# adalca/neurite

Measured on AMD Instinct MI355X. Metric: Mvoxels/sec interpn+Dice on 160^3 x 32-label, higher is better.
Workload: dtype f32

## Files before the change

### neurite_amd/csrc/fused.hip

```cpp

#include <stdio.h>
#include <stdlib.h>

#include <type_traits>

#include "dice_reduce.h"
#include "interpn_core.h"
#include "wc.h"
#include "fused_wc.h"

namespace {

typedef unsigned nrt_u2 __attribute__((ext_vector_type(2)));
template <typename ST> struct RowT;
template <> struct RowT<float> {
    typedef nrt_f4 T;
    static constexpr unsigned BYTES = 16;
    static __device__ __forceinline__ nrt_f4 widen(const nrt_f4 &t) { return t; }
};
template <> struct RowT<unsigned short> {
    typedef nrt_u2 T;
    static constexpr unsigned BYTES = 8;
    static __device__ __forceinline__ nrt_f4 widen(const nrt_u2 &t) {
        return (nrt_f4){__uint_as_float(t[0] << 16), __uint_as_float(t[0] & 0xffff0000u), __uint_as_float(t[1] << 16),
                        __uint_as_float(t[1] & 0xffff0000u)};
    }
};


constexpr int FUSED_SYNC = 8;
constexpr int FUSED_MINW = 3;

template <bool BY_VALUE, typename T> using BodyArg = std::conditional_t<BY_VALUE, const T, const T &>;
template <int G, int MODE, bool STORE, typename ST, bool PAD>
__device__ __forceinline__ void warp_dice_tile_body(BodyArg<PAD && MODE == NRT_LOC_LINSPACE && STORE, InterpArgs> a,
                                                    BodyArg<PAD && !std::is_same<ST, float>::value, TileGeom> tg,
                                                    const void *__restrict__ fixed,
                                                    float *__restrict__ fpart, float *__restrict__ mpart, int Gr_arg) {
    typedef typename RowT<ST>::T Row;
    constexpr unsigned RB = RowT<ST>::BYTES;
    constexpr int NG = 256 / G;
    constexpr int LP = 4 * G;
    const int Gr = PAD ? Gr_arg : G;
    const int L = 4 * Gr;
    const unsigned k = blockIdx.x % NRT_NXCD, jb = blockIdx.x / NRT_NXCD;
    unsigned per = tg.per2 * tg.nTz;
    unsigned nb = gridDim.x / NRT_NXCD;
    int b = blockIdx.y;
    unsigned ucol = 0, prow = blockIdx.x;
    XmWork xw = {};
// ... 237 lines not shown
    if (t == 0 && G == 8 && xmarch_applies(out_shape, batch)) {
        t = xmarch_default_tune();
        tile_geometry(out_shape, G, t, t, tg, nblocks);
    }
    if (((t >> 14) & 1) && !tg.plane_major) {
        int lty = tg.lty;
        while ((1 << (lty + tg.ltz)) < 256 / G) ++lty;
        if (lty != tg.lty) {
            t = (t & ~((15 << 4) | (15 << 8))) | (lty << 4) | (tg.ltz << 8);
            tile_geometry(out_shape, G, t, t, tg, nblocks);
        }
    }
    if (nblocks > (unsigned)DICE_MAX_BLOCKS) nblocks = DICE_MAX_BLOCKS;
    if (((t >> 14) & 1) && !tg.plane_major && out_shape[0] > 0) {
        unsigned grid;
        if (((t >> 16) & 0xff) == 0) nblocks = xmarch_setup_mixed(out_shape, batch, t, tg, grid);
        else nblocks = xmarch_setup(out_shape, batch, t, tg);
    }
}

constexpr int FUSED_TUNE_WC = 1 << 29, FUSED_TUNE_NO_WC = 1 << 30;

struct FusedChoice { bool wc, persist; };
inline FusedChoice fused_choose(const InterpArgs &a, const TileGeom &tg, int G, bool f32_storage, bool allow_wc) {
    FusedChoice c = {false, false};
    if (G == 8 && f32_storage && allow_wc && wc_applies(tg, G, a)) {
        c.wc = true;
        c.persist = wc_persistent(tg);
    }
    return c;
}

template <typename... P, typename... A>
int launch_kernel(void (*kern)(P...), dim3 grid, unsigned dyn, hipStream_t st, A... args) {
    if (dyn && hipFuncSetAttribute((const void *)kern, hipFuncAttributeMaxDynamicSharedMemorySize, (int)dyn) != hipSuccess)
        return NRT_ERR_LAUNCH;
    hipLaunchKernelGGL(kern, grid, dim3(256), dyn, st, args...);
    return NRT_OK;
}

template <int G, int MODE, bool STORE, int MINW, typename ST, bool PAD>
int launch_tile(dim3 grid, unsigned dyn, hipStream_t st, const InterpArgs &a, const TileGeom &tg, const void *fixed, float *fpart,
                float *mpart, int Gr) {
    if constexpr (PAD) return launch_kernel(warp_dice_tile_pad<G, MODE, STORE, MINW, ST>, grid, dyn, st, a, tg, fixed, fpart, mpart, Gr);
    else return launch_kernel(warp_dice_tile<G, MODE, STORE, MINW, ST>, grid, dyn, st, a, tg, fixed, fpart, mpart);
}

template <int G, typename ST, bool PAD>
int launch_fused(const InterpArgs &a, const TileGeom &tg, unsigned nblocks, int batch, int mode, bool store, int Gr,
                 const void *fixed, float *fpart, float *mpart, hipStream_t st, bool allow_wc, bool want_minmax) {
    if constexpr (G == 8 && std::is_same<ST, float>::value && !PAD) {
        if (fused_choose(a, tg, G, true, allow_wc).wc)
            return launch_wc(a, tg, nblocks, batch, mode, store, want_minmax, (const float *)fixed, fpart, mpart, st);
    }
    const dim3 grid = tg.x_march ? dim3(fused_xmarch_grid(tg, nblocks, batch), 1) : dim3(nblocks, batch);
    const unsigned dyn = tg.x_march && !store ? 75u * 1024u : 0u;
#define NRT_FUSED(MODE)                                                                                                          \
    return tg.x_march ? (store ? launch_tile<G, MODE, true, FUSED_MINW, ST, PAD>(grid, dyn, st, a, tg, fixed, fpart, mpart, Gr)  \
                               : launch_tile<G, MODE, false, FUSED_MINW, ST, PAD>(grid, dyn, st, a, tg, fixed, fpart, mpart, Gr)) \
                      : (store ? launch_tile<G, MODE, true, 1, ST, PAD>(grid, dyn, st, a, tg, fixed, fpart, mpart, Gr)           \
                               : launch_tile<G, MODE, false, 1, ST, PAD>(grid, dyn, st, a, tg, fixed, fpart, mpart, Gr))
    switch (mode) {
        case NRT_LOC_ABSOLUTE: NRT_FUSED(NRT_LOC_ABSOLUTE);
        case NRT_LOC_SHIFT: NRT_FUSED(NRT_LOC_SHIFT);
        default: NRT_FUSED(NRT_LOC_LINSPACE);
    }
#undef NRT_FUSED
}

template <int G, typename ST, typename... A>
int launch_fused_any(int Gr, const A &...args) {
    if constexpr (G > 1) {
        if (Gr != G) return launch_fused<G, ST, true>(args...);
    }
    return launch_fused<G, ST, false>(args...);
}
// ... 125 lines not shown
```

### neurite_amd/csrc/fused_wc.h

```cpp

#pragma once

#include <type_traits>

#include "dice_reduce.h"
#include "interpn_core.h"

namespace {

#ifndef WC_NST_WARP
#define WC_NST_WARP 3
#endif
#ifndef WC_NST_FUSED
#define WC_NST_FUSED 2
#endif
#ifndef WC_NST_BWD
#define WC_NST_BWD 3
#endif
#ifndef WC_FIXED_GROUPS
#define WC_FIXED_GROUPS 4
#endif
constexpr int WC_SLOTS = 128;
constexpr int WC_OVF = 16;
constexpr int WC_TRASH_ROW = WC_SLOTS + WC_OVF;
constexpr int WC_ROWS = WC_TRASH_ROW + 1;
constexpr unsigned WC_NOROW = 0x01ffffffu;
constexpr unsigned WC_TAGS_OFF = WC_ROWS * 128;
constexpr unsigned WC_LIST_OFF = WC_TAGS_OFF + 528;
constexpr unsigned WC_BC_OFF = WC_LIST_OFF + 512;
constexpr unsigned WC_WAVE_BYTES = WC_BC_OFF + 128;
constexpr unsigned WC_BLOCK_BYTES = 4 * WC_WAVE_BYTES;
static_assert(WC_LIST_OFF % 16 == 0 && WC_BC_OFF % 16 == 0 && WC_WAVE_BYTES % 16 == 0, "LDS layout");
static_assert((WC_SLOTS + 1) * 4 <= 528 && WC_ROWS <= 256, "LDS layout");
static_assert(2 * WC_BLOCK_BYTES <= 160 * 1024, "two blocks per CU");

typedef __attribute__((address_space(3))) char wc_lds_char;
typedef __attribute__((address_space(3))) nrt_f4 wc_lds_f4;
typedef __attribute__((address_space(3))) volatile nrt_i4 wc_lds_vi4;
typedef __attribute__((address_space(3))) volatile unsigned wc_lds_vu32;
typedef unsigned wc_u3 __attribute__((ext_vector_type(3)));
typedef unsigned wc_u4 __attribute__((ext_vector_type(4)));
typedef float wc_f3 __attribute__((ext_vector_type(3)));

__device__ __forceinline__ void wc_corner(float pv, float mx, int &i0, int &i1, float &w0) {
    const float cl = fminf(fmaxf(pv, 0.0f), mx);
    const float l0 = floorf(cl);
    const float l1 = fminf(nrt_add(l0, 1.0f), mx);
    i0 = (int)l0; i1 = (int)l1;
    w0 = nrt_sub(l1, cl);
}

__device__ __forceinline__ __amdgpu_buffer_rsrc_t wc_rsrc(const void *base, unsigned bytes) {
    const unsigned long long v = (unsigned long long)base;
    const void *u = (const void *)(((unsigned long long)(unsigned)__builtin_amdgcn_readfirstlane((unsigned)(v >> 32)) << 32) |
                                   (unsigned long long)(unsigned)__builtin_amdgcn_readfirstlane((unsigned)v));
    return __builtin_amdgcn_make_buffer_rsrc((void *)u, 0, __builtin_amdgcn_readfirstlane((int)bytes), 0x00020000);
}

struct WcBwd {
    const float *sums, *gdice;
    float eps;
    float *gloc;
};

template <int MODE, bool STORE, bool MM, bool FILL, bool DICE, int BWD = 0>
__device__ __forceinline__ void wc_item(const InterpArgs &a, const TileGeom &tg, const float *__restrict__ fixed, float *__restrict__ fpart,
                                        float *__restrict__ mpart, const XmWork &xw, char *wc_smem, const WcBwd &bw = WcBwd{nullptr, nullptr, 0.0f, nullptr}) {
    constexpr int G = 8, L = 32;
    static_assert(BWD == 0 || (DICE && !STORE && !MM), "the backward form reads a second row per voxel and stores the location gradient only");
    const int b = __builtin_amdgcn_readfirstlane(xw.b);
    const unsigned prow = (unsigned)__builtin_amdgcn_readfirstlane((int)xw.prow), ucol = (unsigned)__builtin_amdgcn_readfirstlane((int)xw.ucol);
    const unsigned RY = 1u << tg.lry, RZ = 1u << tg.lrz;
    const unsigned nRz = (tg.nTz + RZ - 1) / RZ;
    const unsigned reg = ucol / (RY * RZ), wr = ucol % (RY * RZ);
    const unsigned cy = (reg / nRz) * RY + wr / RZ, cz = (reg % nRz) * RZ + wr % RZ;
    const int x0 = __builtin_amdgcn_readfirstlane(xw.x0), y0 = (int)cy << 2, z0 = (int)cz << 3;
    int npass = __builtin_amdgcn_readfirstlane(xw.xlen);
    if (cy >= tg.nTy || cz >= tg.nTz || npass < 0) npass = 0;

    const int lane = threadIdx.x & 63, wave = threadIdx.x >> 6;
    const int g = lane >> 3, p = lane & 7;
    const int dzt = (0x1320 >> ((g & 3) * 4)) & 15;
    const int yy = y0 + 2 * (wave >> 1) + (g >> 2), zz = z0 + 4 * (wave & 1) + dzt;
    const bool yzvalid = (yy < a.O[1]) && (zz < a.O[2]);
    const int yc = min(yy, a.O[1] - 1), zc = min(zz, a.O[2] - 1);
    const unsigned qyz = (unsigned)yc * (unsigned)a.O[2] + (unsigned)zc, qstep = (unsigned)a.O[1] * (unsigned)a.O[2];
    const unsigned SY = (unsigned)a.S[1], SZ = (unsigned)a.S[2];
    const float mxx = (float)(a.S[0] - 1), mxy = (float)(a.S[1] - 1), mxz = (float)(a.S[2] - 1);
    const float fyc = (float)yc, fzc = (float)zc;
    const float ly = (yc == 0) ? 0.0f : ((yc == a.O[1] - 1) ? mxy : nrt_mul(a.delta[1], fyc));
    const float lz = (zc == 0) ? 0.0f : ((zc == a.O[2] - 1) ? mxz : nrt_mul(a.delta[2], fzc));

    const char *volb = (const char *)a.vol + (long long)b * a.vol_bs * 4ll;
    const unsigned long long volbytes = (unsigned long long)a.S[0] * SY * SZ * 128ull;
    const unsigned outbytes = a.nout * 128u;
    const __amdgpu_buffer_rsrc_t vres = wc_rsrc(volb, (unsigned)volbytes);
    const __amdgpu_buffer_rsrc_t lres = wc_rsrc(MODE != NRT_LOC_LINSPACE ? (const char *)(a.loc + (long long)b * a.loc_bs) : volb, a.nout * 12u);
    const __amdgpu_buffer_rsrc_t fres = wc_rsrc(DICE ? (const char *)fixed + (long long)b * a.out_bs * 4ll : volb, outbytes);
    const __amdgpu_buffer_rsrc_t ores = wc_rsrc(STORE ? (const char *)a.out + (long long)b * a.out_bs * 4ll : volb, outbytes);
    const __amdgpu_buffer_rsrc_t gres = wc_rsrc(BWD ? (const char *)(bw.gloc + (long long)b * a.nout * 3) : volb, a.nout * 12u);
    const unsigned gl_lane = (p == 0 && yzvalid) ? qyz * 12u : 0xffffffffu;
    float ca[4] = {0.0f, 0.0f, 0.0f, 0.0f}, cb[4] = {0.0f, 0.0f, 0.0f, 0.0f};
    if (BWD == 1) {
        const float *sm = bw.sums + (long long)b * 3 * L;
#pragma unroll
        for (int k = 0; k < 4; ++k) {
            const int l = p * 4 + k;
            const float num = 2.0f * sm[l] + bw.eps, den = sm[L + l] + sm[2 * L + l] + bw.eps;
            const float gd = bw.gdice[(long long)b * L + l];
            if (den != 0.0f) { ca[k] = 2.0f * gd / den; cb[k] = -2.0f * gd * num / (den * den); }
        }
    }
    const unsigned loc_lane = qyz * 12u, row_lane = (qyz * 8u + (unsigned)p) * 16u;
    const unsigned out_lane = yzvalid ? row_lane : 0xffffffffu;
    const unsigned loc_step = qstep * 12u, row_step = qstep * 128u;
    const unsigned p16 = (unsigned)p * 16u;

    wc_lds_char *wl = (wc_lds_char *)wc_smem + wave * WC_WAVE_BYTES;
    wc_lds_vu32 *tags = (wc_lds_vu32 *)(wl + WC_TAGS_OFF);
    wc_lds_char *lrow = wl + p * 16;
    tags[lane] = ~0u;
    tags[lane + 64] = ~0u;
    const bool cx1 = (p & 4) != 0, cy1 = (p & 2) != 0, cz1 = (p & 1) != 0;

    nrt_f2 stp_l = {0, 0}, stp_h = {0, 0}, stt_l = {0, 0}, stt_h = {0, 0}, spp_l = {0, 0}, spp_h = {0, 0};
    float mnt = INFINITY, mxt = -INFINITY, mnp = INFINITY, mxp = -INFINITY;

    constexpr int FG = WC_FIXED_GROUPS, NX = 8 - FG;
    static_assert(FG == 3 || FG == 4, "WC_FIXED_GROUPS");
    struct Pass {
        float w0x, w0y, w0z;
        unsigned sl[8];
        unsigned lr[FG], ld[FG];
        unsigned xr[NX], xd[NX];
        int n;
        int xq;
        float mk[3];
        bool oob;
        nrt_f4 T;
        nrt_f4 F[FG], Fx[NX];
        float pn[3];
    };
    struct Mg { float w0x, w0y, w0z; bool oob, miss; unsigned rid, slot, t1, t2, mytag; float mk[3]; };
    constexpr int NST = ((BWD ? WC_NST_BWD : (DICE ? WC_NST_FUSED : WC_NST_WARP)) > 2) ? 3 : 2;
    constexpr bool XSH = NST == 3 && DICE;
    Pass A, B, C;
    nrt_f4 FxS[NX];
#pragma unroll
    for (int i = 0; i < NX; ++i) FxS[i] = (nrt_f4){0.f, 0.f, 0.f, 0.f};
    auto reset = [&](Pass &s) {
        s.w0x = s.w0y = s.w0z = 0.f; s.n = 0; s.xq = x0; s.oob = false; s.mk[0] = s.mk[1] = s.mk[2] = 0.f;
        s.T = (nrt_f4){0.f, 0.f, 0.f, 0.f};
#pragma unroll
        for (int i = 0; i < FG; ++i) { s.F[i] = (nrt_f4){0.f, 0.f, 0.f, 0.f}; s.lr[i] = WC_NOROW << 7; s.ld[i] = WC_TRASH_ROW * 128u; }
#pragma unroll
        for (int i = 0; i < NX; ++i) { s.Fx[i] = (nrt_f4){0.f, 0.f, 0.f, 0.f}; s.xr[i] = WC_NOROW << 7; s.xd[i] = WC_TRASH_ROW * 128u; }
#pragma unroll
        for (int i = 0; i < 8; ++i) s.sl[i] = 0;
        s.pn[0] = s.pn[1] = s.pn[2] = 0.f;
    };
    reset(A); reset(B);
    if (NST == 3) reset(C);

    auto fetch_loc = [&](int pass, Pass &s) {
        if (MODE != NRT_LOC_LINSPACE) {
            const wc_u3 v = __builtin_bit_cast(wc_u3, __builtin_amdgcn_raw_buffer_load_b96(lres, loc_lane, (unsigned)(x0 + pass) * loc_step, 0));
            s.pn[0] = __uint_as_float(v[0]); s.pn[1] = __uint_as_float(v[1]); s.pn[2] = __uint_as_float(v[2]);
        }
    };
    auto fetch_row = [&](unsigned rowoff) -> nrt_f4 {
        return __builtin_bit_cast(nrt_f4, __builtin_amdgcn_raw_buffer_load_b128(vres, rowoff | p16, 0, 0));
    };

    auto m1a = [&](int pass, const Pass &s, Mg &m) {
        const int xq = x0 + pass;
        float px, py, pz;
        if (MODE == NRT_LOC_ABSOLUTE) { px = s.pn[0]; py = s.pn[1]; pz = s.pn[2]; }
        else if (MODE == NRT_LOC_SHIFT) { px = nrt_add((float)xq, s.pn[0]); py = nrt_add(fyc, s.pn[1]); pz = nrt_add(fzc, s.pn[2]); }
        else { px = (xq == 0) ? 0.0f : ((xq == a.O[0] - 1) ? mxx : nrt_mul(a.delta[0], (float)xq)); py = ly; pz = lz; }
        int i0x, i1x, i0y, i1y, i0z, i1z;
        wc_corner(px, mxx, i0x, i1x, m.w0x);
        wc_corner(py, mxy, i0y, i1y, m.w0y);
        wc_corner(pz, mxz, i0z, i1z, m.w0z);
        m.oob = FILL ? ((px < 0.0f) || (px > mxx) || (py < 0.0f) || (py > mxy) || (pz < 0.0f) || (pz > mxz)) : false;
        if (BWD) {
            m.mk[0] = (fminf(fmaxf(px, 0.0f), mxx) == px) ? 1.0f : 0.0f;
            m.mk[1] = (fminf(fmaxf(py, 0.0f), mxy) == py) ? 1.0f : 0.0f;
            m.mk[2] = (fminf(fmaxf(pz, 0.0f), mxz) == pz) ? 1.0f : 0.0f;
        }
        const unsigned ix = cx1 ? i1x : i0x, iy = cy1 ? i1y : i0y, iz = cz1 ? i1z : i0z;
        m.rid = nrt_mad24(nrt_mad24(ix, SY, iy), SZ, iz);
        m.slot = ((ix & 3u) << 5) | ((iy & 3u) << 3) | (iz & 7u);
        m.mytag = (m.rid << 6) | (unsigned)lane;
        m.t1 = tags[m.slot];
// ... 6 lines not shown
    auto m1c = [&](int pass, const Mg &m, Pass &s) {
        const unsigned x2 = m.t2 ^ m.mytag;
        const bool served = x2 < 64u;
        const bool loader = m.miss && x2 == 0u;
        const bool orphan = !served;
        const unsigned long long Ml = __builtin_amdgcn_ballot_w64(loader), Mo = __builtin_amdgcn_ballot_w64(orphan);
        const unsigned long long Mf = Ml | Mo;
        const int no = __builtin_popcountll(Mo);
        int n = __builtin_popcountll(Mf);
        const unsigned ro = __builtin_amdgcn_mbcnt_hi((unsigned)(Mo >> 32), __builtin_amdgcn_mbcnt_lo((unsigned)Mo, 0u));
        const unsigned rf = __builtin_amdgcn_mbcnt_hi((unsigned)(Mf >> 32), __builtin_amdgcn_mbcnt_lo((unsigned)Mf, 0u));
        bool fetcher = loader || orphan;
        unsigned src = orphan ? (unsigned)WC_SLOTS + ro : m.slot;
        unsigned e = fetcher ? rf : (unsigned)n + ((unsigned)lane - rf);
        if (__builtin_expect(no > WC_OVF, 0)) {
            tags[lane] = ~0u;
            tags[lane + 64] = ~0u;
            e = (unsigned)lane; fetcher = true; src = (unsigned)lane; n = 64;
        }
        const unsigned src128 = src * 128u;
        const unsigned tp = ((e & 7u) << 3) | (e >> 3);
        typedef unsigned wc_u2 __attribute__((ext_vector_type(2)));
        *(__attribute__((address_space(3))) volatile wc_u2 *)(wl + WC_LIST_OFF + tp * 8u) =
            (wc_u2){fetcher ? (m.rid << 7) : (WC_NOROW << 7), fetcher ? src128 : (unsigned)WC_TRASH_ROW * 128u};
        ((__attribute__((address_space(3))) volatile unsigned short *)(wl + WC_BC_OFF))[lane] = (unsigned short)src128;
        const nrt_i4 la = *(wc_lds_vi4 *)(wl + WC_LIST_OFF + g * 64), lb = *(wc_lds_vi4 *)(wl + WC_LIST_OFF + g * 64 + 16);
        const nrt_i4 sh = *(wc_lds_vi4 *)(wl + WC_BC_OFF + g * 16);
        s.lr[0] = (unsigned)la[0]; s.ld[0] = (unsigned)la[1]; s.lr[1] = (unsigned)la[2]; s.ld[1] = (unsigned)la[3];
        s.lr[2] = (unsigned)lb[0]; s.ld[2] = (unsigned)lb[1];
        if (FG == 4) { s.lr[FG - 1] = (unsigned)lb[2]; s.ld[FG - 1] = (unsigned)lb[3]; }
        else { s.xr[0] = (unsigned)lb[2]; s.xd[0] = (unsigned)lb[3]; }
        if (__builtin_expect(n > 32, 0)) {
            const nrt_i4 lc = *(wc_lds_vi4 *)(wl + WC_LIST_OFF + g * 64 + 32), le = *(wc_lds_vi4 *)(wl + WC_LIST_OFF + g * 64 + 48);
            s.xr[NX - 4] = (unsigned)lc[0]; s.xd[NX - 4] = (unsigned)lc[1]; s.xr[NX - 3] = (unsigned)lc[2]; s.xd[NX - 3] = (unsigned)lc[3];
            s.xr[NX - 2] = (unsigned)le[0]; s.xd[NX - 2] = (unsigned)le[1]; s.xr[NX - 1] = (unsigned)le[2]; s.xd[NX - 1] = (unsigned)le[3];
        }
#pragma unroll
        for (int c = 0; c < 4; ++c) { s.sl[2 * c] = (unsigned)sh[c] & 0xffffu; s.sl[2 * c + 1] = (unsigned)sh[c] >> 16; }
        s.w0x = m.w0x; s.w0y = m.w0y; s.w0z = m.w0z; s.oob = m.oob;
        s.n = __builtin_amdgcn_readfirstlane(n);
        if (BWD) { s.mk[0] = m.mk[0]; s.mk[1] = m.mk[1]; s.mk[2] = m.mk[2]; }
        s.xq = x0 + pass;
    };
    auto issue = [&](Pass &s) {
#pragma unroll
        for (int i = 0; i < FG; ++i) s.F[i] = fetch_row(s.lr[i]);
        if (!XSH && __builtin_expect(s.n > 8 * FG, 0)) {
#pragma unroll
            for (int i = 0; i < NX; ++i)
                if (i == 0 || s.n > 8 * (FG + i)) s.Fx[i] = fetch_row(s.xr[i]);
        }
        if (DICE) s.T = __builtin_bit_cast(nrt_f4, __builtin_amdgcn_raw_buffer_load_b128(fres, row_lane, (unsigned)s.xq * row_step, 2));
    };
    auto issue_x = [&](Pass &s) {
        if (XSH && __builtin_expect(s.n > 8 * FG, 0)) {
#pragma unroll
            for (int i = 0; i < NX; ++i)
                if (i == 0 || s.n > 8 * (FG + i)) FxS[i] = fetch_row(s.xr[i]);
        }
    };
    auto deliver = [&](Pass &s) {
        *(wc_lds_f4 *)(lrow + s.ld[0]) = s.F[0];
#pragma unroll
        for (int i = 1; i < FG; ++i)
            if (s.n > 8 * i) *(wc_lds_f4 *)(lrow + s.ld[i]) = s.F[i];
        if (__builtin_expect(s.n > 8 * FG, 0)) {
#pragma unroll
            for (int i = 0; i < NX; ++i)
                if (i == 0 || s.n > 8 * (FG + i)) *(wc_lds_f4 *)(lrow + s.xd[i]) = XSH ? FxS[i] : s.Fx[i];
        }
    };

    const int last = npass - 1;
    auto step = [&](int pass, Pass &s, Pass &o, Pass &nx, auto masked) {
        constexpr bool MASKED = decltype(masked)::value;
        issue(o);
        __builtin_amdgcn_sched_barrier(0);
        deliver(s);
        nrt_f4 R[8];
#pragma unroll
        for (int corner = 0; corner < 8; ++corner) R[corner] = *(const wc_lds_f4 *)(lrow + s.sl[corner]);
        __builtin_amdgcn_sched_barrier(0);
        Mg m;
        m1a(min(pass + NST, last), s, m);
        __builtin_amdgcn_sched_barrier(0);
        const float w1x = nrt_sub(1.0f, s.w0x), w1y = nrt_sub(1.0f, s.w0y), w1z = nrt_sub(1.0f, s.w0z);
        const nrt_f2 wy2 = {s.w0y, w1y}, wz2 = {s.w0z, w1z};
        const nrt_f2 wxy0 = (nrt_f2){s.w0x, s.w0x} * wy2, wxy1 = (nrt_f2){w1x, w1x} * wy2;
        nrt_f2 wt2[4];
        wt2[0] = (nrt_f2){wxy0[0], wxy0[0]} * wz2;
        wt2[1] = (nrt_f2){wxy0[1], wxy0[1]} * wz2;
        wt2[2] = (nrt_f2){wxy1[0], wxy1[0]} * wz2;
// ... 9 lines not shown
        }
        asm volatile("" : "+v"(al), "+v"(ah));
        __builtin_amdgcn_sched_barrier(0);
        m1b(m);
        __builtin_amdgcn_sched_barrier(0);
#pragma unroll
        for (int corner = 4; corner < (BLEND ? 8 : 4); ++corner) {
            const float wt = wt2[corner >> 1][corner & 1];
            const nrt_f2 w2 = {wt, wt};
            al = al + w2 * (nrt_f2){R[corner][0], R[corner][1]};
            ah = ah + w2 * (nrt_f2){R[corner][2], R[corner][3]};
        }
        nrt_f4 acc = {al[0], al[1], ah[0], ah[1]};
        const unsigned xqcur = (unsigned)s.xq;
        const float cw0x = s.w0x, cw0y = s.w0y, cw0z = s.w0z, cmx = s.mk[0], cmy = s.mk[1], cmz = s.mk[2];
        const bool coob = s.oob;
        if (!BWD) {
            if (FILL) {
#pragma unroll
                for (int c = 0; c < 4; ++c) acc[c] = apply_fill(acc[c], s.oob, a.fill_f);
            }
            if (STORE) __builtin_amdgcn_raw_buffer_store_b128(__builtin_bit_cast(wc_u4, acc), ores, out_lane, (unsigned)s.xq * row_step, 2);
        }
        const nrt_f4 Tcur = s.T;
        asm volatile("" : "+v"(acc));
        __builtin_amdgcn_sched_barrier(0);
        m1c(min(pass + NST, last), m, s);
        __builtin_amdgcn_sched_barrier(0);
        if (BWD) {
            nrt_f2 gl2 = {Tcur[0], Tcur[1]}, gh2 = {Tcur[2], Tcur[3]};
            if (BWD == 1) {
                gl2 = __builtin_elementwise_fma((nrt_f2){cb[0], cb[1]}, (nrt_f2){acc[0], acc[1]}, (nrt_f2){ca[0], ca[1]} * gl2);
                gh2 = __builtin_elementwise_fma((nrt_f2){cb[2], cb[3]}, (nrt_f2){acc[2], acc[3]}, (nrt_f2){ca[2], ca[3]} * gh2);
            }
            if (FILL && coob) { gl2 = (nrt_f2){0.0f, 0.0f}; gh2 = gl2; }
            float gacc[3];
            loc_grad_rows(R, gl2, gh2, cw0x, w1x, cw0y, w1y, cw0z, w1z, cmx, cmy, cmz, gacc);
#pragma unroll
            for (int d = 0; d < 3; ++d) {
                float r = gacc[d];
                r += __int_as_float(__builtin_amdgcn_update_dpp(0, __float_as_int(r), 0xB1, 0xF, 0xF, true));
                r += __int_as_float(__builtin_amdgcn_update_dpp(0, __float_as_int(r), 0x4E, 0xF, 0xF, true));
                r += __int_as_float(__builtin_amdgcn_update_dpp(0, __float_as_int(r), 0x141, 0xF, 0xF, true));
                gacc[d] = r;
            }
            __builtin_amdgcn_raw_buffer_store_b96(__builtin_bit_cast(wc_u3, (wc_f3){gacc[0], gacc[1], gacc[2]}), gres, gl_lane, xqcur * loc_step, 0);
        } else if (DICE) {
            nrt_f4 T = Tcur;
            if (MASKED) {
#pragma unroll
                for (int c = 0; c < 4; ++c) { T[c] = yzvalid ? T[c] : 0.0f; acc[c] = yzvalid ? acc[c] : 0.0f; }
// ... 57 lines not shown
        fetch_loc(min(2, last), A);
        m1a(min(1, last), B, m); m1b(m); m1c(min(1, last), m, B);
        fetch_loc(min(3, last), B);
        __builtin_amdgcn_sched_barrier(0);
        int pass = 0;
        if (npass >= 2) {
            step(0, A, B, B, masked);
            step(1, B, A, A, masked);
            for (pass = 2; pass + 1 < npass; pass += 2) {
                step(pass, A, B, B, masked);
                step(pass + 1, B, A, A, masked);
            }
        }
        if (pass < npass) step(pass, A, B, B, masked);
    };
    if (npass > 0) {
        if (DICE && !BWD && __builtin_amdgcn_ballot_w64(!yzvalid) != 0ull) march(std::true_type());
        else march(std::false_type());
    }

    if (!DICE || BWD) return;
    nrt_f4 stp = {stp_l[0], stp_l[1], stp_h[0], stp_h[1]}, stt = {stt_l[0], stt_l[1], stt_h[0], stt_h[1]},
           spp = {spp_l[0], spp_l[1], spp_h[0], spp_h[1]};
#pragma unroll
    for (int c = 0; c < 4; ++c) {
        stp[c] = wave_xor_add(stp[c], G);
        stt[c] = wave_xor_add(stt[c], G);
        spp[c] = wave_xor_add(spp[c], G);
    }
    for (int off = 1; off < NRT_WAVE; off <<= 1) {
        mnt = fminf(mnt, __shfl_xor(mnt, off, NRT_WAVE)); mxt = fmaxf(mxt, __shfl_xor(mxt, off, NRT_WAVE));
        mnp = fminf(mnp, __shfl_xor(mnp, off, NRT_WAVE)); mxp = fmaxf(mxp, __shfl_xor(mxp, off, NRT_WAVE));
    }
    __syncthreads();
    float (*red)[3 * L + 4] = (float (*)[3 * L + 4])wc_smem;
    if (lane < G) {
#pragma unroll
        for (int c = 0; c < 4; ++c) {
            red[wave][0 * L + 4 * lane + c] = stp[c];
            red[wave][1 * L + 4 * lane + c] = stt[c];
            red[wave][2 * L + 4 * lane + c] = spp[c];
        }
    }
    if (lane == 0) { red[wave][3 * L + 0] = mnt; red[wave][3 * L + 1] = mxt; red[wave][3 * L + 2] = mnp; red[wave][3 * L + 3] = mxp; }
    __syncthreads();
    const long long pbase = (long long)b * tg.prows + prow;
// ... 33 lines not shown
        if (jb == 0xffffffffu) break;
        XmWork xw;
        if (!xmarch_work_at(tg, O0, kk, jb, xw)) continue;
        item(xw);
    }
    if (threadIdx.x == 0 && atomicAdd(&queue[NRT_NXCD * 16u], 1u) == gridDim.x - 1) {
        for (unsigned q = 0; q <= NRT_NXCD; ++q) queue[q * 16u] = 0u;
    }
}

template <int MODE, bool STORE, bool MM, bool FILL, bool DICE = true, bool PERSIST = false>
__global__ __launch_bounds__(256, 2) void warp_dice_wc(InterpArgs a, TileGeom tg, const float *__restrict__ fixed,
                                                        float *__restrict__ fpart, float *__restrict__ mpart, unsigned *__restrict__ queue) {
    extern __shared__ __attribute__((aligned(16))) char wc_smem[];
    if (!PERSIST) {
        XmWork xw;
        if (!xmarch_work(tg, a.O[0], xw)) return;
        wc_item<MODE, STORE, MM, FILL, DICE>(a, tg, fixed, fpart, mpart, xw, wc_smem);
        return;
    }
    wc_persistent_loop(tg, a.O[0], queue, [&](const XmWork &xw) { wc_item<MODE, STORE, MM, FILL, DICE>(a, tg, fixed, fpart, mpart, xw, wc_smem); });
}

template <int MODE, bool FILL, int BWD, bool PERSIST>
__global__ __launch_bounds__(256, 2) void warp_dice_wc_bwd(InterpArgs a, TileGeom tg, const float *__restrict__ rows, WcBwd bw,
                                                            unsigned *__restrict__ queue) {
    extern __shared__ __attribute__((aligned(16))) char wc_smem[];
    if (!PERSIST) {
        XmWork xw;
        if (!xmarch_work(tg, a.O[0], xw)) return;
        wc_item<MODE, false, false, FILL, true, BWD>(a, tg, rows, nullptr, nullptr, xw, wc_smem, bw);
        return;
    }
    wc_persistent_loop(tg, a.O[0], queue, [&](const XmWork &xw) { wc_item<MODE, false, false, FILL, true, BWD>(a, tg, rows, nullptr, nullptr, xw, wc_smem, bw); });
}

inline bool wc_persistent(const TileGeom &tg) { return NRT_NXCD * tg.items_x > 2u * (unsigned)nrt_num_cus(); }
static_assert(NRT_RING_GATHER_OFF == 0 && (NRT_NXCD + 1) * 16 <= NRT_RING_CCE_OFF, "the work counters of a launch stay in the gather's words of a slot");

template <int MODE, bool STORE, bool MM, bool FILL>
int launch_wc_inst(const InterpArgs &a, const TileGeom &tg, unsigned nblocks, int batch, const float *fixed, float *fpart, float *mpart,
                   hipStream_t st) {
    const unsigned items = NRT_NXCD * tg.items_x, slots = 2u * (unsigned)nrt_num_cus();
    unsigned *queue = wc_persistent(tg) ? nrt_ring_slot(st) : nullptr;
    if (queue) {
        if (hipFuncSetAttribute((const void *)warp_dice_wc<MODE, STORE, MM, FILL, true, true>, hipFuncAttributeMaxDynamicSharedMemorySize,
                                (int)WC_BLOCK_BYTES) != hipSuccess)
            return NRT_ERR_LAUNCH;
        hipLaunchKernelGGL((warp_dice_wc<MODE, STORE, MM, FILL, true, true>), dim3(nrt_xcd_grid(slots)), dim3(256), WC_BLOCK_BYTES, st, a, tg, fixed,
                           fpart, mpart, queue);
        return NRT_OK;
    }
    if (hipFuncSetAttribute((const void *)warp_dice_wc<MODE, STORE, MM, FILL>, hipFuncAttributeMaxDynamicSharedMemorySize, (int)WC_BLOCK_BYTES) != hipSuccess)
        return NRT_ERR_LAUNCH;
    hipLaunchKernelGGL((warp_dice_wc<MODE, STORE, MM, FILL>), dim3(items), dim3(256), WC_BLOCK_BYTES, st, a, tg, fixed, fpart, mpart,
                       (unsigned *)nullptr);
    (void)nblocks; (void)batch;
    return NRT_OK;
}

template <int MODE, bool FILL>
int launch_wc_fill(const InterpArgs &a, const TileGeom &tg, unsigned nblocks, int batch, bool store, bool minmax, const float *fixed,
                   float *fpart, float *mpart, hipStream_t st) {
    if (store) return minmax ? launch_wc_inst<MODE, true, true, FILL>(a, tg, nblocks, batch, fixed, fpart, mpart, st)
                             : launch_wc_inst<MODE, true, false, FILL>(a, tg, nblocks, batch, fixed, fpart, mpart, st);
    return minmax ? launch_wc_inst<MODE, false, true, FILL>(a, tg, nblocks, batch, fixed, fpart, mpart, st)
                  : launch_wc_inst<MODE, false, false, FILL>(a, tg, nblocks, batch, fixed, fpart, mpart, st);
}

template <int MODE>
int launch_wc_mode(const InterpArgs &a, const TileGeom &tg, unsigned nblocks, int batch, bool store, bool minmax, const float *fixed,
                   float *fpart, float *mpart, hipStream_t st) {
    return a.has_fill ? launch_wc_fill<MODE, true>(a, tg, nblocks, batch, store, minmax, fixed, fpart, mpart, st)
                      : launch_wc_fill<MODE, false>(a, tg, nblocks, batch, store, minmax, fixed, fpart, mpart, st);
}

inline bool wc_applies(const TileGeom &tg, int G, const InterpArgs &a) {
    return tg.x_march && G == 8 && tg.lty == 2 && tg.ltz == 3 && !tg.plane_major &&
           (unsigned long long)a.S[0] * a.S[1] * a.S[2] * 128ull < 0xffffff00ull;
}

inline int launch_wc(const InterpArgs &a, const TileGeom &tg, unsigned nblocks, int batch, int mode, bool store, bool minmax,
                     const float *fixed, float *fpart, float *mpart, hipStream_t st) {
    switch (mode) {
        case NRT_LOC_ABSOLUTE: return launch_wc_mode<NRT_LOC_ABSOLUTE>(a, tg, nblocks, batch, store, minmax, fixed, fpart, mpart, st);
        case NRT_LOC_SHIFT: return launch_wc_mode<NRT_LOC_SHIFT>(a, tg, nblocks, batch, store, minmax, fixed, fpart, mpart, st);
        default: return launch_wc_mode<NRT_LOC_LINSPACE>(a, tg, nblocks, batch, store, minmax, fixed, fpart, mpart, st);
    }
}

template <int MODE, bool FILL>
int launch_wc_interpn_inst(const InterpArgs &a, const TileGeom &tg, hipStream_t st) {
    const unsigned items = NRT_NXCD * tg.items_x, slots = 2u * (unsigned)nrt_num_cus();
    unsigned *queue = (items > slots) ? nrt_ring_slot(st) : nullptr;
    if (queue) {
        if (hipFuncSetAttribute((const void *)warp_dice_wc<MODE, true, false, FILL, false, true>, hipFuncAttributeMaxDynamicSharedMemorySize,
                                (int)WC_BLOCK_BYTES) != hipSuccess)
            return NRT_ERR_LAUNCH;
        hipLaunchKernelGGL((warp_dice_wc<MODE, true, false, FILL, false, true>), dim3(nrt_xcd_grid(slots)), dim3(256), WC_BLOCK_BYTES, st, a, tg,
                           (const float *)nullptr, (float *)nullptr, (float *)nullptr, queue);
        return NRT_OK;
    }
    if (hipFuncSetAttribute((const void *)warp_dice_wc<MODE, true, false, FILL, false>, hipFuncAttributeMaxDynamicSharedMemorySize,
                            (int)WC_BLOCK_BYTES) != hipSuccess)
        return NRT_ERR_LAUNCH;
    hipLaunchKernelGGL((warp_dice_wc<MODE, true, false, FILL, false>), dim3(items), dim3(256), WC_BLOCK_BYTES, st, a, tg, (const float *)nullptr,
                       (float *)nullptr, (float *)nullptr, (unsigned *)nullptr);
    return NRT_OK;
}

// ... 74 lines not shown
```

Measured before the change: 21100.

## Extend the LDS row-cache interpolation+Dice kernel to bf16-stored label maps

Templates the wave-cache kernel on the storage type so bf16 (unsigned short) volumes and fixed maps use 8-byte row loads, widened to f32 before the LDS delivery. A bf16 fused-forward kernel is added with its own block-level Dice reduction, and launch dispatch routes non-float storage to it instead of the generic tile path. This halves the global bytes fetched per row for bf16 inputs. It adds widening work and a separate LDS-based reduction, and the bound check for applying the cache changes. The f32 benchmark path should compile to the same code, which the added ISA comparison script is meant to confirm.

```diff
diff --git a/neurite_amd/csrc/fused.hip b/neurite_amd/csrc/fused.hip
--- a/neurite_amd/csrc/fused.hip
+++ b/neurite_amd/csrc/fused.hip
@@ -10,22 +10,6 @@
 #include "fused_wc.h"
 
 namespace {
-
-typedef unsigned nrt_u2 __attribute__((ext_vector_type(2)));
-template <typename ST> struct RowT;
-template <> struct RowT<float> {
-    typedef nrt_f4 T;
-    static constexpr unsigned BYTES = 16;
-    static __device__ __forceinline__ nrt_f4 widen(const nrt_f4 &t) { return t; }
-};
-template <> struct RowT<unsigned short> {
-    typedef nrt_u2 T;
-    static constexpr unsigned BYTES = 8;
-    static __device__ __forceinline__ nrt_f4 widen(const nrt_u2 &t) {
-        return (nrt_f4){__uint_as_float(t[0] << 16), __uint_as_float(t[0] & 0xffff0000u), __uint_as_float(t[1] << 16),
-                        __uint_as_float(t[1] & 0xffff0000u)};
-    }
-};
 
 
 constexpr int FUSED_SYNC = 8;
@@ -309,9 +293,9 @@
 constexpr int FUSED_TUNE_WC = 1 << 29, FUSED_TUNE_NO_WC = 1 << 30;
 
 struct FusedChoice { bool wc, persist; };
-inline FusedChoice fused_choose(const InterpArgs &a, const TileGeom &tg, int G, bool f32_storage, bool allow_wc) {
+inline FusedChoice fused_choose(const InterpArgs &a, const TileGeom &tg, int G, bool wc_storage, bool allow_wc) {
     FusedChoice c = {false, false};
-    if (G == 8 && f32_storage && allow_wc && wc_applies(tg, G, a)) {
+    if (G == 8 && wc_storage && allow_wc && wc_applies(tg, G, a)) {
         c.wc = true;
         c.persist = wc_persistent(tg);
     }
@@ -336,9 +320,8 @@
 template <int G, typename ST, bool PAD>
 int launch_fused(const InterpArgs &a, const TileGeom &tg, unsigned nblocks, int batch, int mode, bool store, int Gr,
                  const void *fixed, float *fpart, float *mpart, hipStream_t st, bool allow_wc, bool want_minmax) {
-    if constexpr (G == 8 && std::is_same<ST, float>::value && !PAD) {
-        if (fused_choose(a, tg, G, true, allow_wc).wc)
-            return launch_wc(a, tg, nblocks, batch, mode, store, want_minmax, (const float *)fixed, fpart, mpart, st);
+    if constexpr (G == 8 && !PAD) {
+        if (fused_choose(a, tg, G, true, allow_wc).wc) return launch_wc<ST>(a, tg, mode, store, want_minmax, fixed, fpart, mpart, st);
     }
     const dim3 grid = tg.x_march ? dim3(fused_xmarch_grid(tg, nblocks, batch), 1) : dim3(nblocks, batch);
     const unsigned dyn = tg.x_march && !store ? 75u * 1024u : 0u;
diff --git a/neurite_amd/csrc/fused_wc.h b/neurite_amd/csrc/fused_wc.h
--- a/neurite_amd/csrc/fused_wc.h
+++ b/neurite_amd/csrc/fused_wc.h
@@ -42,6 +42,22 @@
 typedef unsigned wc_u4 __attribute__((ext_vector_type(4)));
 typedef float wc_f3 __attribute__((ext_vector_type(3)));
 
+typedef unsigned nrt_u2 __attribute__((ext_vector_type(2)));
+template <typename ST> struct RowT;
+template <> struct RowT<float> {
+    typedef nrt_f4 T;
+    static constexpr unsigned BYTES = 16;
+    static __device__ __forceinline__ nrt_f4 widen(const nrt_f4 &t) { return t; }
+};
+template <> struct RowT<unsigned short> {
+    typedef nrt_u2 T;
+    static constexpr unsigned BYTES = 8;
+    static __device__ __forceinline__ nrt_f4 widen(const nrt_u2 &t) {
+        return (nrt_f4){__uint_as_float(t[0] << 16), __uint_as_float(t[0] & 0xffff0000u), __uint_as_float(t[1] << 16),
+                        __uint_as_float(t[1] & 0xffff0000u)};
+    }
+};
+
 __device__ __forceinline__ void wc_corner(float pv, float mx, int &i0, int &i1, float &w0) {
     const float cl = fminf(fmaxf(pv, 0.0f), mx);
     const float l0 = floorf(cl);
@@ -63,11 +79,16 @@
     float *gloc;
 };
 
-template <int MODE, bool STORE, bool MM, bool FILL, bool DICE, int BWD = 0>
+template <int MODE, bool STORE, bool MM, bool FILL, bool DICE, int BWD = 0, typename ST = float>
 __device__ __forceinline__ void wc_item(const InterpArgs &a, const TileGeom &tg, const float *__restrict__ fixed, float *__restrict__ fpart,
                                         float *__restrict__ mpart, const XmWork &xw, char *wc_smem, const WcBwd &bw = WcBwd{nullptr, nullptr, 0.0f, nullptr}) {
     constexpr int G = 8, L = 32;
     static_assert(BWD == 0 || (DICE && !STORE && !MM), "the backward form reads a second row per voxel and stores the location gradient only");
+    static_assert(std::is_same<ST, float>::value || (DICE && !STORE && BWD == 0), "maps stored in another type: the fused forward only");
+    typedef typename RowT<ST>::T Row;
+    constexpr unsigned RB = RowT<ST>::BYTES, ROWB = 8 * RB;
+    constexpr unsigned LRB = ROWB == 128 ? 7 : 6;
+    static_assert(ROWB == 1u << LRB, "row bytes");
     const int b = __builtin_amdgcn_readfirstlane(xw.b);
     const unsigned prow = (unsigned)__builtin_amdgcn_readfirstlane((int)xw.prow), ucol = (unsigned)__builtin_amdgcn_readfirstlane((int)xw.ucol);
     const unsigned RY = 1u << tg.lry, RZ = 1u << tg.lrz;
@@ -91,12 +112,12 @@
     const float ly = (yc == 0) ? 0.0f : ((yc == a.O[1] - 1) ? mxy : nrt_mul(a.delta[1], fyc));
     const float lz = (zc == 0) ? 0.0f : ((zc == a.O[2] - 1) ? mxz : nrt_mul(a.delta[2], fzc));
 
-    const char *volb = (const char *)a.vol + (long long)b * a.vol_bs * 4ll;
-    const unsigned long long volbytes = (unsigned long long)a.S[0] * SY * SZ * 128ull;
+    const char *volb = (const char *)a.vol + (long long)b * a.vol_bs * (long long)sizeof(ST);
+    const unsigned long long volbytes = (unsigned long long)a.S[0] * SY * SZ * ROWB;
     const unsigned outbytes = a.nout * 128u;
     const __amdgpu_buffer_rsrc_t vres = wc_rsrc(volb, (unsigned)volbytes);
     const __amdgpu_buffer_rsrc_t lres = wc_rsrc(MODE != NRT_LOC_LINSPACE ? (const char *)(a.loc + (long long)b * a.loc_bs) : volb, a.nout * 12u);
-    const __amdgpu_buffer_rsrc_t fres = wc_rsrc(DICE ? (const char *)fixed + (long long)b * a.out_bs * 4ll : volb, outbytes);
+    const __amdgpu_buffer_rsrc_t fres = wc_rsrc(DICE ? (const char *)fixed + (long long)b * a.out_bs * (long long)sizeof(ST) : volb, a.nout * ROWB);
     const __amdgpu_buffer_rsrc_t ores = wc_rsrc(STORE ? (const char *)a.out + (long long)b * a.out_bs * 4ll : volb, outbytes);
     const __amdgpu_buffer_rsrc_t gres = wc_rsrc(BWD ? (const char *)(bw.gloc + (long long)b * a.nout * 3) : volb, a.nout * 12u);
     const unsigned gl_lane = (p == 0 && yzvalid) ? qyz * 12u : 0xffffffffu;
@@ -114,7 +135,8 @@
     const unsigned loc_lane = qyz * 12u, row_lane = (qyz * 8u + (unsigned)p) * 16u;
     const unsigned out_lane = yzvalid ? row_lane : 0xffffffffu;
     const unsigned loc_step = qstep * 12u, row_step = qstep * 128u;
-    const unsigned p16 = (unsigned)p * 16u;
+    const unsigned p16 = (unsigned)p * RB;
+    const unsigned fix_lane = (qyz * 8u + (unsigned)p) * RB, fix_step = qstep * ROWB;
 
     wc_lds_char *wl = (wc_lds_char *)wc_smem + wave * WC_WAVE_BYTES;
     wc_lds_vu32 *tags = (wc_lds_vu32 *)(wl + WC_TAGS_OFF);
@@ -137,24 +159,24 @@
         int xq;
         float mk[3];
         bool oob;
-        nrt_f4 T;
-        nrt_f4 F[FG], Fx[NX];
+        Row T;
+        Row F[FG], Fx[NX];
         float pn[3];
     };
     struct Mg { float w0x, w0y, w0z; bool oob, miss; unsigned rid, slot, t1, t2, mytag; float mk[3]; };
     constexpr int NST = ((BWD ? WC_NST_BWD : (DICE ? WC_NST_FUSED : WC_NST_WARP)) > 2) ? 3 : 2;
     constexpr bool XSH = NST == 3 && DICE;
     Pass A, B, C;
-    nrt_f4 FxS[NX];
-#pragma unroll
-    for (int i = 0; i < NX; ++i) FxS[i] = (nrt_f4){0.f, 0.f, 0.f, 0.f};
+    Row FxS[NX];
+#pragma unroll
+    for (int i = 0; i < NX; ++i) FxS[i] = Row{};
     auto reset = [&](Pass &s) {
         s.w0x = s.w0y = s.w0z = 0.f; s.n = 0; s.xq = x0; s.oob = false; s.mk[0] = s.mk[1] = s.mk[2] = 0.f;
-        s.T = (nrt_f4){0.f, 0.f, 0.f, 0.f};
-#pragma unroll
-        for (int i = 0; i < FG; ++i) { s.F[i] = (nrt_f4){0.f, 0.f, 0.f, 0.f}; s.lr[i] = WC_NOROW << 7; s.ld[i] = WC_TRASH_ROW * 128u; }
-#pragma unroll
-        for (int i = 0; i < NX; ++i) { s.Fx[i] = (nrt_f4){0.f, 0.f, 0.f, 0.f}; s.xr[i] = WC_NOROW << 7; s.xd[i] = WC_TRASH_ROW * 128u; }
+        s.T = Row{};
+#pragma unroll
+        for (int i = 0; i < FG; ++i) { s.F[i] = Row{}; s.lr[i] = WC_NOROW << LRB; s.ld[i] = WC_TRASH_ROW * 128u; }
+#pragma unroll
+        for (int i = 0; i < NX; ++i) { s.Fx[i] = Row{}; s.xr[i] = WC_NOROW << LRB; s.xd[i] = WC_TRASH_ROW * 128u; }
 #pragma unroll
         for (int i = 0; i < 8; ++i) s.sl[i] = 0;
         s.pn[0] = s.pn[1] = s.pn[2] = 0.f;
@@ -168,8 +190,13 @@
             s.pn[0] = __uint_as_float(v[0]); s.pn[1] = __uint_as_float(v[1]); s.pn[2] = __uint_as_float(v[2]);
         }
     };
-    auto fetch_row = [&](unsigned rowoff) -> nrt_f4 {
-        return __builtin_bit_cast(nrt_f4, __builtin_amdgcn_raw_buffer_load_b128(vres, rowoff | p16, 0, 0));
+    auto fetch_row = [&](unsigned rowoff) -> Row {
+        if constexpr (RB == 16) return __builtin_bit_cast(Row, __builtin_amdgcn_raw_buffer_load_b128(vres, rowoff | p16, 0, 0));
+        else return __builtin_bit_cast(Row, __builtin_amdgcn_raw_buffer_load_b64(vres, rowoff | p16, 0, 0));
+    };
+    auto fetch_fixed = [&](unsigned xq) -> Row {
+        if constexpr (RB == 16) return __builtin_bit_cast(Row, __builtin_amdgcn_raw_buffer_load_b128(fres, fix_lane, xq * fix_step, 2));
+        else return __builtin_bit_cast(Row, __builtin_amdgcn_raw_buffer_load_b64(fres, fix_lane, xq * fix_step, 2));
     };
 
     auto m1a = [&](int pass, const Pass &s, Mg &m) {
@@ -222,7 +249,7 @@
         const unsigned tp = ((e & 7u) << 3) | (e >> 3);
         typedef unsigned wc_u2 __attribute__((ext_vector_type(2)));
         *(__attribute__((address_space(3))) volatile wc_u2 *)(wl + WC_LIST_OFF + tp * 8u) =
-            (wc_u2){fetcher ? (m.rid << 7) : (WC_NOROW << 7), fetcher ? src128 : (unsigned)WC_TRASH_ROW * 128u};
+            (wc_u2){fetcher ? (m.rid << LRB) : (WC_NOROW << LRB), fetcher ? src128 : (unsigned)WC_TRASH_ROW * 128u};
         ((__attribute__((address_space(3))) volatile unsigned short *)(wl + WC_BC_OFF))[lane] = (unsigned short)src128;
         const nrt_i4 la = *(wc_lds_vi4 *)(wl + WC_LIST_OFF + g * 64), lb = *(wc_lds_vi4 *)(wl + WC_LIST_OFF + g * 64 + 16);
         const nrt_i4 sh = *(wc_lds_vi4 *)(wl + WC_BC_OFF + g * 16);
@@ -250,7 +277,7 @@
             for (int i = 0; i < NX; ++i)
                 if (i == 0 || s.n > 8 * (FG + i)) s.Fx[i] = fetch_row(s.xr[i]);
         }
-        if (DICE) s.T = __builtin_bit_cast(nrt_f4, __builtin_amdgcn_raw_buffer_load_b128(fres, row_lane, (unsigned)s.xq * row_step, 2));
+        if (DICE) s.T = fetch_fixed((unsigned)s.xq);
     };
     auto issue_x = [&](Pass &s) {
         if (XSH && __builtin_expect(s.n > 8 * FG, 0)) {
@@ -260,14 +287,14 @@
         }
     };
     auto deliver = [&](Pass &s) {
-        *(wc_lds_f4 *)(lrow + s.ld[0]) = s.F[0];
+        *(wc_lds_f4 *)(lrow + s.ld[0]) = RowT<ST>::widen(s.F[0]);
 #pragma unroll
         for (int i = 1; i < FG; ++i)
-            if (s.n > 8 * i) *(wc_lds_f4 *)(lrow + s.ld[i]) = s.F[i];
+            if (s.n > 8 * i) *(wc_lds_f4 *)(lrow + s.ld[i]) = RowT<ST>::widen(s.F[i]);
         if (__builtin_expect(s.n > 8 * FG, 0)) {
 #pragma unroll
             for (int i = 0; i < NX; ++i)
-                if (i == 0 || s.n > 8 * (FG + i)) *(wc_lds_f4 *)(lrow + s.xd[i]) = XSH ? FxS[i] : s.Fx[i];
+                if (i == 0 || s.n > 8 * (FG + i)) *(wc_lds_f4 *)(lrow + s.xd[i]) = RowT<ST>::widen(XSH ? FxS[i] : s.Fx[i]);
         }
     };
 
@@ -323,11 +350,12 @@
             }
             if (STORE) __builtin_amdgcn_raw_buffer_store_b128(__builtin_bit_cast(wc_u4, acc), ores, out_lane, (unsigned)s.xq * row_step, 2);
         }
-        const nrt_f4 Tcur = s.T;
+        const Row Traw = s.T;
         asm volatile("" : "+v"(acc));
         __builtin_amdgcn_sched_barrier(0);
         m1c(min(pass + NST, last), m, s);
         __builtin_amdgcn_sched_barrier(0);
+        const nrt_f4 Tcur = RowT<ST>::widen(Traw);
         if (BWD) {
             nrt_f2 gl2 = {Tcur[0], Tcur[1]}, gh2 = {Tcur[2], Tcur[3]};
             if (BWD == 1) {
@@ -431,6 +459,43 @@
     if (!DICE || BWD) return;
     nrt_f4 stp = {stp_l[0], stp_l[1], stp_h[0], stp_h[1]}, stt = {stt_l[0], stt_l[1], stt_h[0], stt_h[1]},
            spp = {spp_l[0], spp_l[1], spp_h[0], spp_h[1]};
+    if constexpr (!std::is_same<ST, float>::value) {
+        for (int off = 1; off < NRT_WAVE; off <<= 1) {
+            mnt = fminf(mnt, __shfl_xor(mnt, off, NRT_WAVE)); mxt = fmaxf(mxt, __shfl_xor(mxt, off, NRT_WAVE));
+            mnp = fminf(mnp, __shfl_xor(mnp, off, NRT_WAVE)); mxp = fmaxf(mxp, __shfl_xor(mxp, off, NRT_WAVE));
+        }
+        __syncthreads();
+        float *vs = (float *)wc_smem, *wm = vs + 32 * 3 * L;
+        static_assert((32 * 3 * L + 16) * 4 <= WC_BLOCK_BYTES, "reduction scratch");
+        {
+            const int vy = 2 * (wave >> 1) + (g >> 2), vz = 4 * (wave & 1) + dzt;
+            float *mine = vs + (vy * 8 + vz) * 3 * L + 4 * p;
+            *(nrt_f4 *)(mine + 0 * L) = stp;
+            *(nrt_f4 *)(mine + 1 * L) = stt;
+            *(nrt_f4 *)(mine + 2 * L) = spp;
+        }
+        if (lane == 0) { wm[wave * 4 + 0] = mnt; wm[wave * 4 + 1] = mxt; wm[wave * 4 + 2] = mnp; wm[wave * 4 + 3] = mxp; }
+        __syncthreads();
+        const long long prow_b = (long long)b * tg.prows + prow;
+        if (threadIdx.x < 3 * L) {
+            float s = 0.0f;
+#pragma unroll
+            for (int y = 0; y < 4; ++y) {
+                const float *r = vs + y * 8 * 3 * L + threadIdx.x;
+                const float t = ((r[0 * 3 * L] + r[1 * 3 * L]) + (r[2 * 3 * L] + r[3 * 3 * L])) +
+                                ((r[4 * 3 * L] + r[5 * 3 * L]) + (r[6 * 3 * L] + r[7 * 3 * L]));
+                s = y ? s + t : t;
+            }
+            fpart[prow_b * 3 * L + threadIdx.x] = s;
+        }
+        if (threadIdx.x < 4) {
+            float m = wm[threadIdx.x];
+            for (int w2 = 1; w2 < 4; ++w2) m = (threadIdx.x & 1) ? fmaxf(m, wm[w2 * 4 + threadIdx.x]) : fminf(m, wm[w2 * 4 + threadIdx.x]);
+            mpart[prow_b * 4 + threadIdx.x] = m;
+        }
+        xmarch_zero_rows(tg, xw, 3 * L, fpart, mpart);
+        return;
+    }
 #pragma unroll
     for (int c = 0; c < 4; ++c) {
         stp[c] = wave_xor_add(stp[c], G);
@@ -510,6 +575,21 @@
     wc_persistent_loop(tg, a.O[0], queue, [&](const XmWork &xw) { wc_item<MODE, STORE, MM, FILL, DICE>(a, tg, fixed, fpart, mpart, xw, wc_smem); });
 }
 
+template <int MODE, bool MM, bool FILL, bool PERSIST, typename ST>
+__global__ __launch_bounds__(256, 2) void warp_dice_wc_st(InterpArgs a, TileGeom tg, const void *__restrict__ fixed,
+                                                           float *__restrict__ fpart, float *__restrict__ mpart, unsigned *__restrict__ queue) {
+    extern __shared__ __attribute__((aligned(16))) char wc_smem[];
+    static_assert(!std::is_same<ST, float>::value, "float maps: warp_dice_wc");
+    if (!PERSIST) {
+        XmWork xw;
+        if (!xmarch_work(tg, a.O[0], xw)) return;
+        wc_item<MODE, false, MM, FILL, true, 0, ST>(a, tg, (const float *)fixed, fpart, mpart, xw, wc_smem);
+        return;
+    }
+    wc_persistent_loop(tg, a.O[0], queue,
+                       [&](const XmWork &xw) { wc_item<MODE, false, MM, FILL, true, 0, ST>(a, tg, (const float *)fixed, fpart, mpart, xw, wc_smem); });
+}
+
 template <int MODE, bool FILL, int BWD, bool PERSIST>
 __global__ __launch_bounds__(256, 2) void warp_dice_wc_bwd(InterpArgs a, TileGeom tg, const float *__restrict__ rows, WcBwd bw,
                                                             unsigned *__restrict__ queue) {
@@ -526,54 +606,57 @@
 inline bool wc_persistent(const TileGeom &tg) { return NRT_NXCD * tg.items_x > 2u * (unsigned)nrt_num_cus(); }
 static_assert(NRT_RING_GATHER_OFF == 0 && (NRT_NXCD + 1) * 16 <= NRT_RING_CCE_OFF, "the work counters of a launch stay in the gather's words of a slot");
 
-template <int MODE, bool STORE, bool MM, bool FILL>
-int launch_wc_inst(const InterpArgs &a, const TileGeom &tg, unsigned nblocks, int batch, const float *fixed, float *fpart, float *mpart,
-                   hipStream_t st) {
+template <typename K, typename FX>
+int wc_launch_one(K kern, unsigned grid, hipStream_t st, const InterpArgs &a, const TileGeom &tg, FX fixed, float *fpart, float *mpart,
+                  unsigned *queue) {
+    if (hipFuncSetAttribute((const void *)kern, hipFuncAttributeMaxDynamicSharedMemorySize, (int)WC_BLOCK_BYTES) != hipSuccess) return NRT_ERR_LAUNCH;
+    hipLaunchKernelGGL(kern, dim3(grid), dim3(256), WC_BLOCK_BYTES, st, a, tg, fixed, fpart, mpart, queue);
+    return NRT_OK;
+}
+
+template <int MODE, bool STORE, bool MM, bool FILL, typename ST>
+int launch_wc_inst(const InterpArgs &a, const TileGeom &tg, const void *fixed, float *fpart, float *mpart, hipStream_t st) {
     const unsigned items = NRT_NXCD * tg.items_x, slots = 2u * (unsigned)nrt_num_cus();
     unsigned *queue = wc_persistent(tg) ? nrt_ring_slot(st) : nullptr;
-    if (queue) {
-        if (hipFuncSetAttribute((const void *)warp_dice_wc<MODE, STORE, MM, FILL, true, true>, hipFuncAttributeMaxDynamicSharedMemorySize,
-                                (int)WC_BLOCK_BYTES) != hipSuccess)
-            return NRT_ERR_LAUNCH;
-        hipLaunchKernelGGL((warp_dice_wc<MODE, STORE, MM, FILL, true, true>), dim3(nrt_xcd_grid(slots)), dim3(256), WC_BLOCK_BYTES, st, a, tg, fixed,
-                           fpart, mpart, queue);
-        return NRT_OK;
-    }
-    if (hipFuncSetAttribute((const void *)warp_dice_wc<MODE, STORE, MM, FILL>, hipFuncAttributeMaxDynamicSharedMemorySize, (int)WC_BLOCK_BYTES) != hipSuccess)
-        return NRT_ERR_LAUNCH;
-    hipLaunchKernelGGL((warp_dice_wc<MODE, STORE, MM, FILL>), dim3(items), dim3(256), WC_BLOCK_BYTES, st, a, tg, fixed, fpart, mpart,
-                       (unsigned *)nullptr);
-    (void)nblocks; (void)batch;
-    return NRT_OK;
-}
-
-template <int MODE, bool FILL>
-int launch_wc_fill(const InterpArgs &a, const TileGeom &tg, unsigned nblocks, int batch, bool store, bool minmax, const float *fixed,
-                   float *fpart, float *mpart, hipStream_t st) {
-    if (store) return minmax ? launch_wc_inst<MODE, true, true, FILL>(a, tg, nblocks, batch, fixed, fpart, mpart, st)
-                             : launch_wc_inst<MODE, true, false, FILL>(a, tg, nblocks, batch, fixed, fpart, mpart, st);
-    return minmax ? launch_wc_inst<MODE, false, true, FILL>(a, tg, nblocks, batch, fixed, fpart, mpart, st)
-                  : launch_wc_inst<MODE, false, false, FILL>(a, tg, nblocks, batch, fixed, fpart, mpart, st);
-}
-
-template <int MODE>
-int launch_wc_mode(const InterpArgs &a, const TileGeom &tg, unsigned nblocks, int batch, bool store, bool minmax, const float *fixed,
-                   float *fpart, float *mpart, hipStream_t st) {
-    return a.has_fill ? launch_wc_fill<MODE, true>(a, tg, nblocks, batch, store, minmax, fixed, fpart, mpart, st)
-                      : launch_wc_fill<MODE, false>(a, tg, nblocks, batch, store, minmax, fixed, fpart, mpart, st);
+    if constexpr (std::is_same<ST, float>::value) {
+        if (queue)
+            return wc_launch_one(warp_dice_wc<MODE, STORE, MM, FILL, true, true>, nrt_xcd_grid(slots), st, a, tg, (const float *)fixed, fpart, mpart, queue);
+        return wc_launch_one(warp_dice_wc<MODE, STORE, MM, FILL>, items, st, a, tg, (const float *)fixed, fpart, mpart, (unsigned *)nullptr);
+    } else {
+        if constexpr (STORE) return NRT_ERR_UNSUPPORTED;
+        else {
+            if (queue) return wc_launch_one(warp_dice_wc_st<MODE, MM, FILL, true, ST>, nrt_xcd_grid(slots), st, a, tg, fixed, fpart, mpart, queue);
+            return wc_launch_one(warp_dice_wc_st<MODE, MM, FILL, false, ST>, items, st, a, tg, fixed, fpart, mpart, (unsigned *)nullptr);
+        }
+    }
+}
+
+template <int MODE, bool FILL, typename ST>
+int launch_wc_fill(const InterpArgs &a, const TileGeom &tg, bool store, bool minmax, const void *fixed, float *fpart, float *mpart, hipStream_t st) {
+    if (store) return minmax ? launch_wc_inst<MODE, true, true, FILL, ST>(a, tg, fixed, fpart, mpart, st)
+                             : launch_wc_inst<MODE, true, false, FILL, ST>(a, tg, fixed, fpart, mpart, st);
+    return minmax ? launch_wc_inst<MODE, false, true, FILL, ST>(a, tg, fixed, fpart, mpart, st)
+                  : launch_wc_inst<MODE, false, false, FILL, ST>(a, tg, fixed, fpart, mpart, st);
+}
+
+template <int MODE, typename ST>
+int launch_wc_mode(const InterpArgs &a, const TileGeom &tg, bool store, bool minmax, const void *fixed, float *fpart, float *mpart, hipStream_t st) {
+    return a.has_fill ? launch_wc_fill<MODE, true, ST>(a, tg, store, minmax, fixed, fpart, mpart, st)
+                      : launch_wc_fill<MODE, false, ST>(a, tg, store, minmax, fixed, fpart, mpart, st);
 }
 
 inline bool wc_applies(const TileGeom &tg, int G, const InterpArgs &a) {
     return tg.x_march && G == 8 && tg.lty == 2 && tg.ltz == 3 && !tg.plane_major &&
-           (unsigned long long)a.S[0] * a.S[1] * a.S[2] * 128ull < 0xffffff00ull;
-}
-
-inline int launch_wc(const InterpArgs &a, const TileGeom &tg, unsigned nblocks, int batch, int mode, bool store, bool minmax,
-                     const float *fixed, float *fpart, float *mpart, hipStream_t st) {
+           (unsigned long long)a.S[0] * a.S[1] * a.S[2] < (unsigned long long)(WC_NOROW - 1u);
+}
+
+template <typename ST>
+int launch_wc(const InterpArgs &a, const TileGeom &tg, int mode, bool store, bool minmax, const void *fixed, float *fpart, float *mpart,
+              hipStream_t st) {
     switch (mode) {
-        case NRT_LOC_ABSOLUTE: return launch_wc_mode<NRT_LOC_ABSOLUTE>(a, tg, nblocks, batch, store, minmax, fixed, fpart, mpart, st);
-        case NRT_LOC_SHIFT: return launch_wc_mode<NRT_LOC_SHIFT>(a, tg, nblocks, batch, store, minmax, fixed, fpart, mpart, st);
-        default: return launch_wc_mode<NRT_LOC_LINSPACE>(a, tg, nblocks, batch, store, minmax, fixed, fpart, mpart, st);
+        case NRT_LOC_ABSOLUTE: return launch_wc_mode<NRT_LOC_ABSOLUTE, ST>(a, tg, store, minmax, fixed, fpart, mpart, st);
+        case NRT_LOC_SHIFT: return launch_wc_mode<NRT_LOC_SHIFT, ST>(a, tg, store, minmax, fixed, fpart, mpart, st);
+        default: return launch_wc_mode<NRT_LOC_LINSPACE, ST>(a, tg, store, minmax, fixed, fpart, mpart, st);
     }
 }
 
diff --git a/profiles/wc_bf16/isa_compare.py b/profiles/wc_bf16/isa_compare.py
--- /dev/null
+++ b/profiles/wc_bf16/isa_compare.py
@@ -0,0 +1,81 @@
+#!/usr/bin/env python3
+import hashlib
+import os
+import re
+import subprocess
+import sys
+
+
+def kernels(path):
+    out, name, body = {}, None, []
+    desc, dname = {}, None
+    for line in open(path):
+        s = line.strip()
+        m = re.match(r'\.type\s+(\S+),@function', s)
+        if m:
+            name, body = m.group(1), []
+            continue
+        m = re.match(r'\.amdhsa_kernel\s+(\S+)', s)
+        if m:
+            dname = m.group(1)
+            desc[dname] = []
+            continue
+        if s == '.end_amdhsa_kernel':
+            dname = None
+            continue
+        if dname is not None:
+            desc[dname].append(s)
+            continue
+        if name is None:
+            continue
+        if re.match(r'\.Lfunc_end\d+:', s):
+            out[name] = body
+            name = None
+            continue
+        if not s or s.startswith(';') or s.startswith('.p2align') or s == name + ':':
+            continue
+        s = re.sub(r'\s*;.*$', '', s)
+        s = re.sub(r'\.LBB\d+_(\d+)', r'.LBB_\1', s)
+        body.append(s)
+    return {k: (v, desc.get(k, [])) for k, v in out.items()}
+
+
+def demangle(names):
+    rocm = os.environ.get('ROCM_PATH', '/opt/rocm')
+    for tool in ('llvm-cxxfilt', os.path.join(rocm, 'llvm', 'bin', 'llvm-cxxfilt'), 'c++filt'):
+        try:
+            r = subprocess.run([tool], input='\n'.join(names), capture_output=True, text=True, timeout=120)
+            d = r.stdout.split('\n')
+            if r.returncode == 0 and len(d) >= len(names):
+                return dict(zip(names, d))
+        except (OSError, subprocess.SubprocessError):
+            pass
+    return {n: n for n in names}
+
+
+def main():
+    a, b = kernels(sys.argv[1]), kernels(sys.argv[2])
+    dm = demangle(sorted(set(a) | set(b)))
+    short = lambda n: re.sub(r'\(anonymous namespace\)::', '', dm[n]).split('(')[0].replace('void ', '')
+    bad = 0
+    for n in sorted(a):
+        ins, desc = a[n]
+        h = hashlib.sha256('\n'.join(ins).encode()).hexdigest()[:12]
+        if n not in b:
+            state = 'MISSING'
+        elif b[n][0] != ins:
+            state = 'DIFFERENT STREAM (%d -> %d instructions)' % (len(ins), len(b[n][0]))
+        elif b[n][1] != desc:
+            state = 'DIFFERENT DESCRIPTOR'
+        else:
+            state = 'identical'
+        bad += state != 'identical'
+        print('%-24s %6d lines  sha %s  %s' % (state, len(ins), h, short(n)))
+    for n in sorted(set(b) - set(a)):
+        print('%-24s %6d lines  sha %s  %s' % ('new', len(b[n][0]), hashlib.sha256('\n'.join(b[n][0]).encode()).hexdigest()[:12], short(n)))
+    print('%d kernels of the first listing, %d not identical, %d new' % (len(a), bad, len(set(b) - set(a))))
+    return 1 if bad else 0
+
+
+if __name__ == '__main__':
+    sys.exit(main())
```

Result: slower. 20730 (-1.7%).
